# gstoica27/ReLUQP-py

Hardware: AMD Instinct MI355X
Metric: QP solves/sec (batch=4096 random dense QPs n=100 m=300) (higher is better)
Workload: dtype f32; 1 GPU; batch=4096/GPU random dense QPs n=100 m=300 (n_eq=25), feasible rand_qp seeds 0.., eps_abs=0.001, cold start, reference defaults; 4 distinct batches in rotation, every solve without dispatch history (= first solve of a fresh handle); global_batch=4096, parallelism=batch-split x1, no collectives, kernel=resident2, tile=same, low_memory=False, fresh_batches=4, dispatch_history=False, rho_window=5

## Files before the change

### reluqp-py_amd/csrc/rqp_resident2.hip

```cpp
#include <cstdio>
#include <cstdlib>
#include <type_traits>
#include <vector>

#include "rqp_common.h"

typedef float f2 __attribute__((ext_vector_type(2)));
typedef _Float16 h2 __attribute__((ext_vector_type(2)));

__device__ __forceinline__ float fma_mix_lo(h2 k, float v, float acc) {
    asm("v_fma_mix_f32 %0, %1, %2, %0 op_sel_hi:[1,0,0]" : "+v"(acc) : "v"(k), "v"(v));
    return acc;
}
__device__ __forceinline__ float fma_mix_hi(h2 k, float v, float acc) {
    asm("v_fma_mix_f32 %0, %1, %2, %0 op_sel:[1,0,0] op_sel_hi:[1,0,0]" : "+v"(acc) : "v"(k), "v"(v));
    return acc;
}
template <int CTRL>
__device__ __forceinline__ float dpp2(float v) {
    return __builtin_bit_cast(float, __builtin_amdgcn_update_dpp(0, __builtin_bit_cast(int, v), CTRL, 0xF, 0xF, true));
}
__device__ __forceinline__ float swsum32(float a, float b) {
    asm volatile("s_nop 1\n\tv_permlane32_swap_b32 %0, %1" : "+v"(a), "+v"(b));
    return a + b;
}
__device__ __forceinline__ float swsum16(float a, float b) {
    asm volatile("s_nop 1\n\tv_permlane16_swap_b32 %0, %1" : "+v"(a), "+v"(b));
    return a + b;
}
__device__ __forceinline__ float swmax32(float a, float b) {
    asm volatile("s_nop 1\n\tv_permlane32_swap_b32 %0, %1" : "+v"(a), "+v"(b));
    return fmaxf(a, b);
}
__device__ __forceinline__ float swmax16(float a, float b) {
    asm volatile("s_nop 1\n\tv_permlane16_swap_b32 %0, %1" : "+v"(a), "+v"(b));
    return fmaxf(a, b);
}
__device__ __forceinline__ float wave_max(float v) {
    v = fmaxf(v, dpp2<0xB1>(v));
    v = fmaxf(v, dpp2<0x4E>(v));
    v = fmaxf(v, dpp2<0x141>(v));
    v = fmaxf(v, dpp2<0x128>(v));
    float a = v, b = v;
    asm volatile("s_nop 1\n\tv_permlane16_swap_b32 %0, %1" : "+v"(a), "+v"(b));
    v = fmaxf(a, b);
    a = v; b = v;
    asm volatile("s_nop 1\n\tv_permlane32_swap_b32 %0, %1" : "+v"(a), "+v"(b));
    return fmaxf(a, b);
}
__device__ __forceinline__ unsigned wave_or(unsigned v) {
    v |= (unsigned)__builtin_amdgcn_update_dpp(0, (int)v, 0xB1, 0xF, 0xF, true);
    v |= (unsigned)__builtin_amdgcn_update_dpp(0, (int)v, 0x4E, 0xF, 0xF, true);
    v |= (unsigned)__builtin_amdgcn_update_dpp(0, (int)v, 0x141, 0xF, 0xF, true);
    v |= (unsigned)__builtin_amdgcn_update_dpp(0, (int)v, 0x128, 0xF, 0xF, true);
    unsigned a = v, b = v;
    asm volatile("s_nop 1\n\tv_permlane16_swap_b32 %0, %1" : "+v"(a), "+v"(b));
    v = a | b;
    a = v; b = v;
    asm volatile("s_nop 1\n\tv_permlane32_swap_b32 %0, %1" : "+v"(a), "+v"(b));
    return a | b;
}
template <typename T>
__device__ __forceinline__ T tmax2(T a, T b) {
    return (a != a) ? a : ((b != b) ? b : (a > b ? a : b));
}

template <int RB_, int CQ_, int KR_, int KC_>
struct Res2Cfg {
    static constexpr int RB = RB_, CQ = CQ_, KR = KR_, KC = KC_;
    static constexpr int NT = 256, NW = 4, NQ = 2, PL = 32;
    static constexpr int RP = RB / 2, KP = KR / 2;
    static constexpr int CW = NQ * CQ;
    static constexpr int N = NW * CW;
    static constexpr int M = PL * RB;
    static constexpr int SW = 8 * KR + 4;
    static constexpr int ND = NW * SW;
    static constexpr int AE2 = RP * CQ;
    static constexpr int KE2 = KP * KC;
    static constexpr int HR = 4, HP = HR / 2;
    static constexpr int HE2 = HP * CQ;
    static constexpr int HU = HE2 / 2;
    static constexpr int H1 = (CQ + 1) / 2, H2 = (H1 + 1) / 2;
    static constexpr int MATREGS = 2 * (RP * CQ + KP * KC);
    static constexpr int WAVES_PER_SIMD = (MATREGS > 100) ? 2 : ((MATREGS > 30) ? 3 : 4);
    static_assert(RB % 2 == 0 && KR % 2 == 0 && HP == 2 && HU == CQ && PL * HR >= N, "row pairs");
    static_assert(8 * KR >= CW && 8 * KC >= N && M <= 2 * NT && KC == CQ && NQ == 2, "tile shape");
    static constexpr size_t lds_bytes() {
        return (size_t)M * 8 * 4 + ND * 8 + 16 * 8
               + (size_t)M * 4 * 5
               + (size_t)ND * 4 * 6
               + (size_t)NW * M * 4 + 96 * 4
               + (size_t)HU * NT * 16;
    }
};

constexpr int NSEG = 25;
template <class C, bool DIAG, bool KH, bool KD = false>
__global__ void __launch_bounds__(256, C::WAVES_PER_SIMD) k_admm_res2(SolveArgs a, const float* __restrict__ Apack,
                                                      const float* __restrict__ Kpack,
                                                      const float* __restrict__ Hpack, unsigned long long* dbg,
                                                      const float* __restrict__ Kscale) {
    constexpr int RB = C::RB, CQ = C::CQ, KR = C::KR, KC = C::KC, NT = C::NT, NW = C::NW, RP = C::RP, KP = C::KP;
    constexpr int CW = C::CW, M = C::M, ND = C::ND, SW = C::SW, AE2 = C::AE2, KE2 = C::KE2, HU = C::HU, HP = C::HP, HR = C::HR, H1 = C::H1, H2 = C::H2;
    extern __shared__ __attribute__((aligned(16))) unsigned char smem_raw[];
    double* zt64 = (double*)smem_raw;
    double* lam64 = zt64 + M;
    double* z64 = lam64 + M;
    double* inv64 = z64 + M;
    double* x64 = inv64 + M;
    double* redd = x64 + ND;
    float* lT = (float*)(redd + 16);
    float* uT = lT + M;
    float* rv32 = uT + M;
    float* nu = rv32 + M;
    float* cT = nu + M;
    float* xin = cT + M;
    float* xnat = xin + ND;
    float* dxv = xnat + ND;
    float* hx = dxv + ND;
    float* gT = hx + ND;
    float* dvec = gT + ND;
    float* part = dvec + ND;
    float* red = part + NW * M;
    float* Hs = red + 96;
    static_assert(((size_t)M * 8 * 4 + ND * 8 + 16 * 8 + (size_t)M * 4 * 5 + ND * 4 * 6 + NW * M * 4 + 96 * 4) % 16 == 0,
                  "H image must start 16-byte aligned");

    const int n = a.n, m = a.m;
    const int b = a.order ? a.order[blockIdx.x] : (int)blockIdx.x, tid = threadIdx.x;
    const int wave = tid >> 6, lane = tid & 63;
    const int q = lane & 1, pl = lane >> 1, rr = lane >> 3, cc = lane & 7;
    const size_t mat = (a.sA == 0) ? 0 : (size_t)b;
    const float* cg = (const float*)a.c + (size_t)b * m;
    int k0 = 0;
    bool exact = false;
    if (a.cont == 1) {
        if (a.info.status[b] != RQP_STATUS_CONTINUE) {
            if (!(a.warm_starting || a.keep_state)) {
                for (int i = tid; i < n; i += NT) a.x[(size_t)b * n + i] = 0.0;
                for (int i = tid; i < m; i += NT) {
                    a.z[(size_t)b * m + i] = 0.0;
                    a.lam[(size_t)b * m + i] = 0.0;
                }
                if (tid == 0) a.rho_ind[b] = a.rho_ind0;
            }
            return;
        }
        k0 = a.cont_iter[b];
    } else if (a.cont == 2) {
        if (a.gate && *a.gate == 0) return;
        if (a.cstat[b] == 0) return;
        const int ci = a.cont_iter[b];
        if (ci >= 0) {
            k0 = ci;
            exact = true;
        }
    }
    const int wb = a.wbase ? a.wbase[mat] : 0;
    if (a.cstat && a.mode == 0) {
        const int sl = a.rho_ind[b] - wb;
        if (sl < 0 || sl >= a.kwin) {
            if (tid == 0) {
                a.cstat[b] = 1;
                if (!exact) a.cont_iter[b] = -1;
                atomicAdd(a.ncont, 1);
            }
            return;
        }
    }

    f2 ar[RP][CQ];
    {
        const f2* Ap = (const f2*)(Apack + mat * (size_t)AE2 * NT * 2) + tid;
#pragma unroll
        for (int rp = 0; rp < RP; ++rp)
#pragma unroll
            for (int c = 0; c < CQ; ++c) ar[rp][c] = Ap[(size_t)(rp * CQ + c) * NT];
        const float4* Hp = (const float4*)(Hpack + mat * (size_t)HU * NT * 4);
#pragma unroll
        for (int u = 0; u < HU; ++u) ((float4*)Hs)[u * NT + tid] = Hp[u * NT + tid];
    }
    int ri = a.rho_ind[b];
    float* rhoL = red + 64;
    if (tid < 32) rhoL[tid] = (tid < a.nrho) ? (float)a.rhos[tid] : 0.f;
    typedef typename std::conditional<KH, h2, f2>::type kpair_t;
    kpair_t kr[KP][KC];
    float kscale = 1.f;
    auto load_K = [&](int jl) {
        int j = jl - wb;
        j = j < 0 ? 0 : (j >= a.kwin ? a.kwin - 1 : j);
        if constexpr (!KD) {
            int tid_k = tid;
            asm volatile("" : "+v"(tid_k));
            const kpair_t* Kp = (const kpair_t*)Kpack + (mat * a.kwin + j) * (size_t)KE2 * NT + tid_k;
#pragma unroll
            for (int kp = 0; kp < KP; ++kp)
#pragma unroll
                for (int c = 0; c < KC; ++c) kr[kp][c] = Kp[(size_t)(kp * KC + c) * NT];
            if constexpr (KH) kscale = Kscale[mat * a.kwin + j];
        } else {
            int lane_o = lane, wave_o = wave;
            asm volatile("" : "+v"(lane_o), "+v"(wave_o));
            const int rr = lane_o >> 3, cc = lane_o & 7, wave = wave_o;
            const float* Kj = (const float*)a.K + ((a.sK == 0) ? (size_t)0 : (size_t)b * a.sK) + (size_t)j * n * a.ldn;
            typedef float f4u __attribute__((ext_vector_type(4), aligned(4)));
#pragma unroll
            for (int kp = 0; kp < KP; ++kp) {
                const int lr = KR * rr + 2 * kp, r = CW * wave + lr;
                const bool ok0 = lr < CW && r < n, ok1 = lr + 1 < CW && r + 1 < n;
                const float* row0 = Kj + (size_t)(r < n ? r : n - 1) * a.ldn + KC * cc;
                const float* row1 = Kj + (size_t)(r + 1 < n ? r + 1 : n - 1) * a.ldn + KC * cc;
                float t0[KC], t1[KC];
#pragma unroll
                for (int c = 0; c + 4 <= KC; c += 4) {
                    const f4u u0 = *(const f4u*)(row0 + c), u1 = *(const f4u*)(row1 + c);
#pragma unroll
                    for (int e = 0; e < 4; ++e) { t0[c + e] = u0[e]; t1[c + e] = u1[e]; }
                }
#pragma unroll
                for (int c = KC - KC % 4; c < KC; ++c) { t0[c] = row0[c]; t1[c] = row1[c]; }
                const f2 msk = {ok0 ? 1.f : 0.f, ok1 ? 1.f : 0.f};
#pragma unroll
                for (int c = 0; c < KC; ++c) kr[kp][c] = (f2){t0[c], t1[c]} * msk;
            }
        }
    };
    load_K(ri);

    auto set_rho_rows = [&](int j) {
        const float rho = (float)a.rhos[j];
        for (int i = tid; i < M; i += NT) {
            const float rv = rho * ((i < m) ? cg[i] : 1.f);
            rv32[i] = rv;
            inv64[i] = 1.0 / (double)rv;
        }
    };
    for (int i = tid; i < M; i += NT) {
        const bool in = i < m;
        zt64[i] = (exact && in) ? a.ax[(size_t)b * m + i] : 0.0;
        z64[i] = in ? a.z[(size_t)b * m + i] : 0.0;
        lam64[i] = in ? a.lam[(size_t)b * m + i] : 0.0;
        lT[i] = in ? ((const float*)a.l)[(size_t)b * m + i] : 0.f;
        uT[i] = in ? ((const float*)a.u)[(size_t)b * m + i] : 0.f;
        nu[i] = 0.f;
        cT[i] = in ? cg[i] : 1.f;
    }
    set_rho_rows(ri);
    for (int i = tid; i < ND; i += NT) {
        const int col = CW * (i / SW) + (i % SW);
        const bool in = (i % SW) < CW && col < n;
        const double xv = in ? a.x[(size_t)b * n + col] : 0.0;
        x64[i] = xv;
        xin[i] = (float)xv;
        xnat[i] = (i < n) ? (float)a.x[(size_t)b * n + i] : 0.f;
        gT[i] = in ? ((const float*)a.g)[(size_t)b * n + col] : 0.f;
        hx[i] = 0.f;
        dxv[i] = 0.f;
        dvec[i] = 0.f;
    }

    int colw, ncolw;
    {
        const int b5 = (lane >> 5) & 1, b4 = (lane >> 4) & 1;
        const int cbase = H2 * b4 + H1 * b5;
        int nval = b4 ? (H1 - H2) : H2;
        if (b5 && cbase + nval > CQ) nval = CQ - cbase;
        ncolw = ((lane & 0xE) == 0) ? nval : 0;
        colw = SW * wave + CQ * q + cbase;
    }
    __syncthreads();

    auto load_vc = [&](const float* v, float (&vc)[CQ]) __attribute__((always_inline)) {
#pragma unroll
        for (int c = 0; c < CQ; ++c) vc[c] = v[SW * wave + CQ * q + c];
    };
    auto prod_A = [&](const float (&vc)[CQ]) __attribute__((always_inline)) {
        f2 acc[RP];
#pragma unroll
        for (int rp = 0; rp < RP; ++rp) {
            f2 s = {0.f, 0.f};
#pragma unroll
            for (int c = 0; c < CQ; ++c) s = __builtin_elementwise_fma(ar[rp][c], (f2){vc[c], vc[c]}, s);
            s.x += dpp2<0xB1>(s.x);
            s.y += dpp2<0xB1>(s.y);
            acc[rp] = s;
        }
        if (q == 0) {
            f2* dst = (f2*)(part + wave * M + RB * pl);
#pragma unroll
            for (int rp = 0; rp < RP; ++rp) dst[rp] = acc[rp];
        }
    };
    auto prod_At = [&](auto use_a, auto use_h, const float* w, float* out, bool addg) {
        constexpr bool USE_A = decltype(use_a)::value, USE_H = decltype(use_h)::value;
        f2 wr[RP];
        f2 wx[HP];
        if constexpr (USE_A) {
#pragma unroll
            for (int rp = 0; rp < RP; ++rp) wr[rp] = ((const f2*)(w + RB * pl))[rp];
        }
        if constexpr (USE_H) {
            const float4 xv = *(const float4*)(xnat + HR * pl);
            wx[0] = (f2){xv.x, xv.y};
            wx[1] = (f2){xv.z, xv.w};
        }
        auto hload = [&](int c) -> float4 { return ((const float4*)Hs)[c * NT + tid]; };
        auto colsum = [&](int c, const float4& hv) -> float {
            f2 t2 = {0.f, 0.f};
            if constexpr (USE_A) {
#pragma unroll
                for (int rp = 0; rp < RP; ++rp) t2 = __builtin_elementwise_fma(ar[rp][c], wr[rp], t2);
            }
            if constexpr (USE_H) {
                t2 = __builtin_elementwise_fma((f2){hv.x, hv.y}, wx[0], t2);
                t2 = __builtin_elementwise_fma((f2){hv.z, hv.w}, wx[1], t2);
            }
            return t2.x + t2.y;
        };
        float s1[H1];
        auto colsum2 = [&](int c0, int c1, const float4& h0, const float4& h1, float& a0, float& a1) __attribute__((always_inline)) {
            f2 t0 = {0.f, 0.f}, t1 = {0.f, 0.f};
            if constexpr (USE_A) {
#pragma unroll
                for (int rp = 0; rp < RP; ++rp) {
                    t0 = __builtin_elementwise_fma(ar[rp][c0], wr[rp], t0);
                    t1 = __builtin_elementwise_fma(ar[rp][c1], wr[rp], t1);
                }
            }
            if constexpr (USE_H) {
                t0 = __builtin_elementwise_fma((f2){h0.x, h0.y}, wx[0], t0);
                t1 = __builtin_elementwise_fma((f2){h1.x, h1.y}, wx[0], t1);
                t0 = __builtin_elementwise_fma((f2){h0.z, h0.w}, wx[1], t0);
                t1 = __builtin_elementwise_fma((f2){h1.z, h1.w}, wx[1], t1);
            }
            a0 = t0.x + t0.y;
            a1 = t1.x + t1.y;
        };
        float4 hcur = {0.f, 0.f, 0.f, 0.f}, hnext = {0.f, 0.f, 0.f, 0.f};
        if constexpr (USE_H) {
            hcur = hload(0);
            if (H1 < CQ) hnext = hload(H1);
        }
#pragma unroll
        for (int i = 0; i < H1; ++i) {
            const bool pair = (i + H1 < CQ);
            if (pair) {
                float4 hc2 = hcur, hn2 = hnext;
                if constexpr (USE_H) {
                    if (i + 1 < H1) hc2 = hload(i + 1);
                    if (i + 1 + H1 < CQ) hn2 = hload(i + 1 + H1);
                }
                float a0, a1;
                colsum2(i, i + H1, hcur, hnext, a0, a1);
                s1[i] = swsum32(a0, a1);
                hcur = hc2;
                hnext = hn2;
            } else {
                const float a0 = colsum(i, hcur);
                s1[i] = swsum32(a0, a0);
            }
        }
        float gpre[H2];
#pragma unroll
        for (int i = 0; i < H2; ++i) gpre[i] = addg ? gT[colw + i] : 0.f;
        float s2[H2];
#pragma unroll
        for (int i = 0; i < H2; ++i) s2[i] = (i + H2 < H1) ? swsum16(s1[i], s1[i + H2]) : swsum16(s1[i], s1[i]);
#pragma unroll
        for (int i = 0; i < H2; ++i) {
            float v = s2[i];
            v += dpp2<0x4E>(v);
            v += dpp2<0x124>(v);
            v += dpp2<0x128>(v);
            s2[i] = v;
        }
        if (ncolw > 0) {
#pragma unroll
            for (int i = 0; i < H2; ++i)
                if (i < ncolw) out[colw + i] = s2[i] + gpre[i];
        }
    };
    constexpr std::true_type YES{};
    auto prod_At_chk = [&](const float* w, float* outA, float* outH) {
        f2 wr[RP];
        f2 wx[HP];
#pragma unroll
        for (int rp = 0; rp < RP; ++rp) wr[rp] = ((const f2*)(w + RB * pl))[rp];
        {
            const float4 xv = *(const float4*)(xnat + HR * pl);
            wx[0] = (f2){xv.x, xv.y};
            wx[1] = (f2){xv.z, xv.w};
        }
        auto hload = [&](int c) -> float4 { return ((const float4*)Hs)[c * NT + tid]; };
        float sA[H1], sH[H1];
        float4 hcur = hload(0), hnext = {0.f, 0.f, 0.f, 0.f};
        if (H1 < CQ) hnext = hload(H1);
#pragma unroll
        for (int i = 0; i < H1; ++i) {
            const bool pair = (i + H1 < CQ);
            float4 hc2 = hcur, hn2 = hnext;
            if (i + 1 < H1) hc2 = hload(i + 1);
            if (i + 1 + H1 < CQ) hn2 = hload(i + 1 + H1);
            f2 a0 = {0.f, 0.f}, a1 = {0.f, 0.f};
            f2 h0 = __builtin_elementwise_fma((f2){hcur.x, hcur.y}, wx[0], (f2){0.f, 0.f}), h1 = {0.f, 0.f};
            if (pair) h1 = __builtin_elementwise_fma((f2){hnext.x, hnext.y}, wx[0], h1);
#pragma unroll
            for (int rp = 0; rp < RP; ++rp) {
                a0 = __builtin_elementwise_fma(ar[rp][i], wr[rp], a0);
                if (pair) a1 = __builtin_elementwise_fma(ar[rp][i + H1], wr[rp], a1);
            }
            h0 = __builtin_elementwise_fma((f2){hcur.z, hcur.w}, wx[1], h0);
            if (pair) h1 = __builtin_elementwise_fma((f2){hnext.z, hnext.w}, wx[1], h1);
            const float ca0 = a0.x + a0.y, ch0 = h0.x + h0.y;
            sA[i] = pair ? swsum32(ca0, a1.x + a1.y) : swsum32(ca0, ca0);
            sH[i] = pair ? swsum32(ch0, h1.x + h1.y) : swsum32(ch0, ch0);
            hcur = hc2;
            hnext = hn2;
        }
        float tA[H2], tH[H2];
#pragma unroll
        for (int i = 0; i < H2; ++i) {
            tA[i] = (i + H2 < H1) ? swsum16(sA[i], sA[i + H2]) : swsum16(sA[i], sA[i]);
            tH[i] = (i + H2 < H1) ? swsum16(sH[i], sH[i + H2]) : swsum16(sH[i], sH[i]);
        }
#pragma unroll
        for (int i = 0; i < H2; ++i) {
            float va = tA[i], vh = tH[i];
            va += dpp2<0x4E>(va);
            vh += dpp2<0x4E>(vh);
            va += dpp2<0x124>(va);
            vh += dpp2<0x124>(vh);
            va += dpp2<0x128>(va);
            vh += dpp2<0x128>(vh);
            tA[i] = va;
            tH[i] = vh;
        }
        if (ncolw > 0) {
#pragma unroll
            for (int i = 0; i < H2; ++i)
                if (i < ncolw) {
                    outA[colw + i] = tA[i] + 0.f;
                    outH[colw + i] = tH[i] + 0.f;
                }
        }
    };
    auto prod_K = [&](const float* v, float (&s)[KR]) {
        float vc[KC];
#pragma unroll
        for (int c = 0; c < KC; ++c) vc[c] = v[SW * (cc >> 1) + CQ * (cc & 1) + c];
#pragma unroll
        for (int kp = 0; kp < KP; ++kp) {
            f2 t = {0.f, 0.f};
            if constexpr (KH) {
#pragma unroll
                for (int c = 0; c < KC; ++c) {
                    t.x = fma_mix_lo(kr[kp][c], vc[c], t.x);
                    t.y = fma_mix_hi(kr[kp][c], vc[c], t.y);
                }
                t.x *= kscale;
                t.y *= kscale;
            } else {
#pragma unroll
                for (int c = 0; c < KC; ++c) t = __builtin_elementwise_fma(kr[kp][c], (f2){vc[c], vc[c]}, t);
            }
            s[2 * kp] = t.x;
            s[2 * kp + 1] = t.y;
        }
#pragma unroll
        for (int r = 0; r < KR; ++r) s[r] += dpp2<0xB1>(s[r]);
#pragma unroll
        for (int r = 0; r < KR; ++r) s[r] += dpp2<0x4E>(s[r]);
#pragma unroll
        for (int r = 0; r < KR; ++r) s[r] += dpp2<0x141>(s[r]);
    };
    float cv[3] = {0.f, 0.f, 0.f};
    auto row_body = [&](auto nr, bool init, bool do_a, bool do_b, bool chk) __attribute__((always_inline)) {
        constexpr int R = decltype(nr)::value;
        double zt[R], z[R], lmv[R], iv[R];
        float adx[R][NW], lo[R], hi[R], rvf[R];
#pragma unroll
        for (int q = 0; q < R; ++q) {
            const int i = tid + q * NT;
            zt[q] = zt64[i];
            lmv[q] = lam64[i];
            if (do_a) {
                iv[q] = inv64[i];
                lo[q] = lT[i];
                hi[q] = uT[i];
            } else {
                z[q] = z64[i];
            }
            rvf[q] = rv32[i];
            if (init || do_a) {
#pragma unroll
                for (int w = 0; w < NW; ++w) adx[q][w] = part[w * M + i];
            }
        }
        asm volatile("s_waitcnt lgkmcnt(0)" ::: "memory");
#pragma unroll
        for (int q = 0; q < R; ++q) {
            asm volatile("" : "+v"(zt[q]), "+v"(lmv[q]), "+v"(rvf[q]));
            if (do_a) asm volatile("" : "+v"(iv[q]), "+v"(lo[q]), "+v"(hi[q]));
            else asm volatile("" : "+v"(z[q]));
            if (init || do_a) asm volatile("" : "+v"(adx[q][0]), "+v"(adx[q][1]), "+v"(adx[q][2]), "+v"(adx[q][3]));
        }
#pragma unroll
        for (int q = 0; q < R; ++q) {
            const int i = tid + q * NT;
            if (init || do_a) {
                const float ad = ((adx[q][0] + adx[q][1]) + adx[q][2]) + adx[q][3];
                zt[q] = (init ? 0.0 : zt[q]) + (double)ad;
                zt64[i] = zt[q];
            }
            if (do_a) {
                const double v = zt[q] + lmv[q] * iv[q];
                z[q] = v;
                if (v < (double)lo[q]) z[q] = (double)lo[q];
                if (v > (double)hi[q]) z[q] = (double)hi[q];
                z64[i] = z[q];
            }
            if (do_b) {
                const double rv = (double)rvf[q];
                const double pr = zt[q] - z[q];
                const double lh = lmv[q] + rv * pr;
                lam64[i] = lh;
                nu[i] = (float)(lh + rv * pr);
            }
        }
        if (chk) {
            int tid_w = tid;
            asm volatile("" : "+v"(tid_w));
#pragma unroll
            for (int q = 0; q < R; ++q) {
                const int i = tid_w + q * NT;
                const float we = (a.scE && i < m) ? (float)(1.0 / a.scE[mat * m + i]) : 1.f;
                nu[i] = (float)lmv[q];
                cv[0] = tmax2(cv[0], fabsf((float)(zt[q] - z[q])) * we);
                cv[1] = tmax2(cv[1], fabsf((float)zt[q]) * we);
                cv[2] = tmax2(cv[2], fabsf((float)z[q]) * we);
            }
        }
    };
    auto row_pass = [&](bool init, bool do_a, bool do_b, bool chk = false) __attribute__((always_inline)) {
        if constexpr (M > NT) {
            static_assert(M <= 2 * NT, "at most two rows per lane");
            if (tid + NT < M) {
                row_body(std::integral_constant<int, 2>{}, init, do_a, do_b, chk);
                return;
            }
        }
        if (tid < M) row_body(std::integral_constant<int, 1>{}, init, do_a, do_b, chk);
    };

    __builtin_amdgcn_s_waitcnt(0x0F70);
    unsigned long long t_last = 0, t_acc[NSEG] = {};
    bool k_pend = false;
    bool diag_on = true;
    auto stamp = [&](int seg) {
        if constexpr (DIAG) {
            __builtin_amdgcn_sched_barrier(0);
            unsigned long long t;
            asm volatile("s_memtime %0\n\ts_waitcnt lgkmcnt(0)" : "=s"(t)::"memory");
            __builtin_amdgcn_sched_barrier(0);
            if (seg >= 0 && diag_on) t_acc[seg] += t - t_last;
            t_last = t;
        }
    };

    float rho_est = (a.mode == 2) ? (float)a.rho_in : ((a.cont == 1 || exact) ? (float)a.cont_rho[b] : (float)a.rhos[ri]);
    float pri = 0.f, dua = 0.f;
    bool converged = false;
    int iters = k0;
    const float tolT = (float)a.tol;
    const int kmax = (a.mode == 2) ? 0 : a.max_iter;

    if (!exact) {
        float vc0[CQ];
        load_vc(xin, vc0);
        prod_A(vc0);
        __syncthreads();
        row_pass(true, false, kmax > k0);
    } else {
        row_pass(false, false, kmax > k0);
    }

    float scl_p = 0.f, scl_d = 0.f;
    auto res_rows = [&]() {
        cv[0] = cv[1] = cv[2] = 0.f;
        int tid_w = tid;
        asm volatile("" : "+v"(tid_w));
        for (int i = tid_w; i < M; i += NT) {
            const float we = (a.scE && i < m) ? (float)(1.0 / a.scE[mat * m + i]) : 1.f;
            nu[i] = (float)lam64[i];
            cv[0] = tmax2(cv[0], fabsf((float)(zt64[i] - z64[i])) * we);
            cv[1] = tmax2(cv[1], fabsf((float)zt64[i]) * we);
            cv[2] = tmax2(cv[2], fabsf((float)z64[i]) * we);
        }
    };
    int rpar = 0;
    auto residuals = [&](float rho_carry, float& o_pri, float& o_dua) -> float {
        float v[7];
#pragma unroll
        for (int e = 0; e < 3; ++e) v[e] = cv[e];
#pragma unroll
        for (int e = 3; e < 7; ++e) v[e] = 0.f;
        int tid_w = tid;
        asm volatile("" : "+v"(tid_w));
        __syncthreads();
        stamp(10);
        if (tid < ND && (tid % SW) >= CW) {
            dxv[tid] = 0.f;
            hx[tid] = 0.f;
        }
        prod_At_chk(nu, dxv, hx);
        stamp(11);
        __syncthreads();
        stamp(13);
        if (tid < ND) {
            float wd = 1.f;
            if (a.scD) {
                const int col = CW * (tid_w / SW) + (tid_w % SW);
                if ((tid_w % SW) < CW && col < n) wd = (float)(1.0 / (a.scC[mat] * a.scD[mat * n + col]));
            }
            const float t3 = dxv[tid];
            v[3] = fabsf(hx[tid] + t3 + gT[tid]) * wd;
            v[4] = fabsf(hx[tid]) * wd;
            v[5] = fabsf(t3) * wd;
            v[6] = fabsf(gT[tid]) * wd;
        }
        unsigned nanm = 0;
#pragma unroll
        for (int e = 0; e < 7; ++e) nanm |= (__builtin_amdgcn_ballot_w64(v[e] != v[e]) != 0ull) ? (1u << e) : 0u;
        float u0, u1;
        {
            const float r0 = swmax32(v[0], v[4]), r1 = swmax32(v[1], v[5]), r2 = swmax32(v[2], v[6]), r3 = swmax32(v[3], v[3]);
            u0 = swmax16(r0, r2);
            u1 = swmax16(r1, r3);
        }
        u0 = fmaxf(u0, dpp2<0xB1>(u0));
        u1 = fmaxf(u1, dpp2<0xB1>(u1));
        u0 = fmaxf(u0, dpp2<0x4E>(u0));
        u1 = fmaxf(u1, dpp2<0x4E>(u1));
        u0 = fmaxf(u0, dpp2<0x141>(u0));
        u1 = fmaxf(u1, dpp2<0x141>(u1));
        u0 = fmaxf(u0, dpp2<0x128>(u0));
        u1 = fmaxf(u1, dpp2<0x128>(u1));
        float* redp = red + 32 * rpar;
        rpar ^= 1;
        if ((lane & 15) == 0) {
            const int row = lane >> 4;
            *(f2*)(redp + wave * 8 + 2 * row) = (f2){u0, row == 3 ? __builtin_bit_cast(float, nanm) : u1};
        }
        stamp(14);
        __syncthreads();
        stamp(15);
        nanm = 0;
#pragma unroll
        for (int w = 0; w < NW; ++w) nanm |= __builtin_bit_cast(unsigned, redp[w * 8 + 7]);
#pragma unroll
        for (int e = 0; e < 7; ++e) {
            float r = redp[e];
#pragma unroll
            for (int w = 1; w < NW; ++w) r = fmaxf(r, redp[w * 8 + e]);
            v[e] = ((nanm >> e) & 1u) ? __builtin_nanf("") : r;
        }
        stamp(16);
        o_pri = v[0];
        o_dua = v[3];
        scl_p = tmax2(v[1], v[2]);
        scl_d = tmax2(tmax2(v[4], v[5]), v[6]);
        const float num = v[0] / scl_p;
        const float den = v[3] / scl_d;
        float est = rho_carry * sqrtf(num / den);
        if (est < (float)a.rho_min) est = (float)a.rho_min;
        if (est > (float)a.rho_max) est = (float)a.rho_max;
        return est;
    };

    stamp(-1);
    int to_chk = a.check_interval - (k0 % a.check_interval);
    for (int k = k0 + 1; k <= kmax; ++k) {
        __syncthreads();
        stamp(0);
        prod_At(YES, YES, nu, dvec, true);
        stamp(1);
        __syncthreads();
        stamp(2);
        __builtin_amdgcn_s_waitcnt(0x0F70);
        if constexpr (DIAG) {
            if (k_pend) { stamp(20); k_pend = false; }
        }
        {
            float s[KR];
            static_assert(KR == 4 || KR == 2, "vectorised x update");
            const int j = SW * wave + KR * rr;
            double2* xp = (double2*)(x64 + j);
            double2 xold[KR / 2];
#pragma unroll
            for (int hlf = 0; hlf < KR / 2; ++hlf) xold[hlf] = xp[hlf];
            prod_K(dvec, s);
            if (cc == 0) {
#pragma unroll
                for (int hlf = 0; hlf < KR / 2; ++hlf) ((f2*)(dxv + j))[hlf] = (f2){-s[2 * hlf], -s[2 * hlf + 1]};
            }
            __builtin_amdgcn_fence(__ATOMIC_RELEASE, "wavefront");
            __builtin_amdgcn_wave_barrier();
            float vc[CQ];
            load_vc(dxv, vc);
            if (cc == 0) {
                f2* xn2 = (f2*)(xnat + CW * wave + KR * rr);
#pragma unroll
                for (int hlf = 0; hlf < KR / 2; ++hlf) {
                    double2 xa = xold[hlf];
                    const f2 dx = {-s[2 * hlf], -s[2 * hlf + 1]};
                    xa.x += (double)dx.x;
                    xa.y += (double)dx.y;
                    xp[hlf] = xa;
                    const f2 xf = {(float)xa.x, (float)xa.y};
                    ((f2*)(xin + j))[hlf] = xf;
                    if (KR * rr + 2 * hlf + 1 < CW) xn2[hlf] = xf;
                }
            }
            stamp(3);
            prod_A(vc);
        }
        stamp(4);
        __syncthreads();
        stamp(5);
        stamp(6);
        iters = k;
        const bool on_grid = (--to_chk == 0);
        if (on_grid) to_chk = a.check_interval;
        const bool check = (a.mode == 0) && on_grid;
        if (!check) {
            row_pass(false, true, k < kmax);
            stamp(7);
        } else {
            cv[0] = cv[1] = cv[2] = 0.f;
            row_pass(false, true, false, true);
            stamp(8);
            if constexpr (DIAG) t_acc[22] += 1;
            const int ri_before = ri;
            rho_est = residuals(rho_est, pri, dua);
            rho_est = __builtin_bit_cast(float, __builtin_amdgcn_readfirstlane(__builtin_bit_cast(int, rho_est)));
            pri = __builtin_bit_cast(float, __builtin_amdgcn_readfirstlane(__builtin_bit_cast(int, pri)));
            dua = __builtin_bit_cast(float, __builtin_amdgcn_readfirstlane(__builtin_bit_cast(int, dua)));
            if (rho_est > rhoL[ri] * tolT && ri < a.nrho - 1)
                ri += 1;
            else if (rho_est < rhoL[ri] / tolT && ri > 0)
                ri -= 1;
            if (a.info.trace && (k / a.check_interval) <= a.info.trace_cap && tid == 0) {
                double* tr = a.info.trace + ((size_t)b * a.info.trace_cap + (k / a.check_interval - 1)) * 4;
                tr[0] = (double)pri; tr[1] = (double)dua; tr[2] = (double)rho_est; tr[3] = (double)ri_before;
            }
            float tp = (float)a.thr_p, td = (float)a.thr_d;
            if (a.eps_rel > 0) {
                tp += (float)a.eps_rel * __builtin_bit_cast(float, __builtin_amdgcn_readfirstlane(__builtin_bit_cast(int, scl_p)));
                td += (float)a.eps_rel * __builtin_bit_cast(float, __builtin_amdgcn_readfirstlane(__builtin_bit_cast(int, scl_d)));
            }
            stamp(18);
            if (pri < tp && dua < td) {
                converged = true;
                break;
            }
            if (ri != ri_before) {
                if (a.cstat && k < kmax && (ri < wb || ri >= wb + a.kwin)) {
                    int tid_o = tid;
                    asm volatile("" : "+v"(tid_o));
                    for (int i = tid_o; i < n; i += NT) a.x[(size_t)b * n + i] = x64[SW * (i / CW) + i % CW];
                    for (int i = tid_o; i < m; i += NT) {
                        a.z[(size_t)b * m + i] = z64[i];
                        a.lam[(size_t)b * m + i] = lam64[i];
                        a.ax[(size_t)b * m + i] = zt64[i];
                    }
                    if (tid_o == 0) {
                        a.rho_ind[b] = ri;
                        a.cont_iter[b] = k;
                        a.cont_rho[b] = (double)rho_est;
                        a.cstat[b] = 1;
                        atomicAdd(a.ncont, 1);
                    }
                    return;
                }
                if constexpr (DIAG) { t_acc[23] += 1; k_pend = true; }
                if constexpr (!KD) load_K(ri);
                {
                    int tid_o = tid;
                    asm volatile("" : "+v"(tid_o));
                    const float rho = rhoL[ri];
                    for (int i = tid_o; i < M; i += NT) {
                        const float rv = rho * cT[i];
                        rv32[i] = rv;
                        inv64[i] = 1.0 / (double)rv;
                    }
                }
                if constexpr (KD) load_K(ri);
                stamp(19);
            }
            if (k < kmax) row_pass(false, false, true);
            stamp(21);
        }
    }
    if constexpr (DIAG) {
        diag_on = false;
        if (lane == 0)
            for (int e = 0; e < NSEG; ++e) dbg[((size_t)b * 4 + wave) * NSEG + e] = (e == NSEG - 1) ? (unsigned long long)iters : t_acc[e];
    }

    __syncthreads();
    if (a.mode == 1) {
        for (int i = tid; i < n; i += NT) a.x[(size_t)b * n + i] = x64[SW * (i / CW) + i % CW];
        for (int i = tid; i < m; i += NT) {
            a.z[(size_t)b * m + i] = z64[i];
            a.lam[(size_t)b * m + i] = lam64[i];
        }
        return;
    }
    if (!converged) {
        res_rows();
        rho_est = residuals(rho_est, pri, dua);
    }

    double jp = 0.0;
    if (tid < ND) jp = (double)(xin[tid] * (0.5f * hx[tid] + gT[tid]));
    for (int off = 32; off >= 1; off >>= 1) jp += __shfl_xor(jp, off, 64);
    if (lane == 0) redd[wave] = jp;
    __syncthreads();
    const double obj = redd[0] + redd[1] + redd[2] + redd[3];

    if (a.mode == 2) {
        if (tid == 0) {
            if (a.r_pri) a.r_pri[b] = (double)pri;
            if (a.r_dua) a.r_dua[b] = (double)dua;
            if (a.r_rho) a.r_rho[b] = (double)rho_est;
            if (a.r_obj) a.r_obj[b] = obj;
        }
        return;
    }

    if (a.out_x) for (int i = tid; i < n; i += NT) ((float*)a.out_x)[(size_t)b * n + i] = (float)x64[SW * (i / CW) + i % CW];
    if (a.out_z) for (int i = tid; i < m; i += NT) ((float*)a.out_z)[(size_t)b * m + i] = (float)z64[i];
    if (a.out_lam) for (int i = tid; i < m; i += NT) ((float*)a.out_lam)[(size_t)b * m + i] = (float)lam64[i];
    if (tid == 0) {
        if (a.cstat) a.cstat[b] = 0;
        if (a.info.iter) a.info.iter[b] = converged ? iters : a.max_iter;
        if (a.last_iter) a.last_iter[b] = converged ? iters : a.max_iter;
        if (a.info.status) a.info.status[b] = converged ? RQP_STATUS_SOLVED : ((pri != pri || dua != dua) ? RQP_STATUS_NAN : RQP_STATUS_MAX_ITER);
        if (a.info.rho_ind) a.info.rho_ind[b] = ri;
        if (a.info.pri_res) a.info.pri_res[b] = (double)pri;
        if (a.info.dua_res) a.info.dua_res[b] = (double)dua;
        if (a.info.rho_estimate) a.info.rho_estimate[b] = (double)rho_est;
        if (a.info.obj_val) a.info.obj_val[b] = obj;
    }
    if ((a.warm_starting || a.keep_state)) {
        for (int i = tid; i < n; i += NT) a.x[(size_t)b * n + i] = x64[SW * (i / CW) + i % CW];
        for (int i = tid; i < m; i += NT) {
            a.z[(size_t)b * m + i] = z64[i];
            a.lam[(size_t)b * m + i] = lam64[i];
        }
        if (tid == 0) a.rho_ind[b] = ri;
    } else {
        for (int i = tid; i < n; i += NT) a.x[(size_t)b * n + i] = 0.0;
        for (int i = tid; i < m; i += NT) {
            a.z[(size_t)b * m + i] = 0.0;
            a.lam[(size_t)b * m + i] = 0.0;
        }
        if (tid == 0) a.rho_ind[b] = a.rho_ind0;
    }
}

template <class C, bool KH>
__global__ void k_pack_res2(int n, int ldn, int nrho, const float* __restrict__ K, float* __restrict__ Kpack, float* __restrict__ Kscale,
                            const int32_t* __restrict__ only, const int32_t* __restrict__ gate) {
    constexpr int KR = C::KR, KC = C::KC, NT = C::NT, CW = C::CW, KE2 = C::KE2;
    const int mat = blockIdx.y;
    if (gate && *gate == 0) return;
    if (only && !only[mat]) return;
    const int t = threadIdx.x, w = t >> 6, lane = t & 63;
    const int rr = lane >> 3, cc = lane & 7;
    extern __shared__ __attribute__((aligned(16))) float stage[];
    {
        const int j = blockIdx.x;
        const float* Kj = K + ((size_t)mat * nrho + j) * n * ldn;
        for (int i = t; i < n * ldn; i += NT) stage[i] = Kj[i];
        __syncthreads();
        float inv_scale = 1.f;
        if constexpr (KH) {
            __shared__ float smax[NT];
            float mx = 0.f;
            for (int i = t; i < n * ldn; i += NT) mx = fmaxf(mx, fabsf(stage[i]));
            smax[t] = mx;
            __syncthreads();
            for (int off = NT / 2; off >= 1; off >>= 1) {
                if (t < off) smax[t] = fmaxf(smax[t], smax[t + off]);
                __syncthreads();
            }
            int e2 = 0;
            (void)frexpf(fmaxf(smax[0], 1e-30f), &e2);
            const float sc = ldexpf(1.f, e2 - 14);
            inv_scale = ldexpf(1.f, 14 - e2);
            if (t == 0) Kscale[(size_t)mat * nrho + j] = sc;
        }
        float* Kp = Kpack + ((size_t)mat * nrho + j) * KE2 * NT * (KH ? 1 : 2);
        for (int pair = 0; pair < KE2; ++pair) {
            const int lr = KR * rr + 2 * (pair / KC);
            const int r = CW * w + lr, c = KC * cc + pair % KC;
            f2 v;
            v.x = (lr < CW && r < n && c < n) ? stage[r * ldn + c] : 0.f;
            v.y = (lr + 1 < CW && r + 1 < n && c < n) ? stage[(r + 1) * ldn + c] : 0.f;
            if constexpr (KH)
                ((h2*)Kp)[(size_t)pair * NT + t] = (h2){(_Float16)(v.x * inv_scale), (_Float16)(v.y * inv_scale)};
            else
                ((f2*)Kp)[(size_t)pair * NT + t] = v;
        }
    }
}


template <class C>
__global__ void k_pack_res2_ah(int n, int m, int ldn, const float* __restrict__ A, const float* __restrict__ Ht,
                               float* __restrict__ Apack, float* __restrict__ Hpack) {
    constexpr int RB = C::RB, CQ = C::CQ, NT = C::NT, CW = C::CW, AE2 = C::AE2, HU = C::HU, HR = C::HR, RCH = C::M / 4;
    const int mat = blockIdx.y, ch = blockIdx.x, t = threadIdx.x;
    extern __shared__ __attribute__((aligned(16))) float stage[];
    if (ch < 4) {
        if (!A) return;
        const int r0 = RCH * ch;
        const float* Am = A + (size_t)mat * m * ldn + (size_t)r0 * ldn;
        const int avail = (m - r0) * ldn;
        if ((((size_t)Am) & 15) == 0) {
            for (int i = 4 * t; i < RCH * ldn; i += 4 * NT)
                *(float4*)(stage + i) = (i < avail) ? *(const float4*)(Am + i) : (float4){0.f, 0.f, 0.f, 0.f};
        } else {
            for (int i = t; i < RCH * ldn; i += NT) stage[i] = (i < avail) ? Am[i] : 0.f;
        }
        __syncthreads();
        const int l16 = t & 15, w = (t >> 4) & 3, part = t >> 6;
        const int lane = 16 * ch + l16, q = lane & 1, pl = lane >> 1, tk = 64 * w + lane;
        f2* Ap = (f2*)(Apack + (size_t)mat * AE2 * NT * 2);
        for (int pair = part; pair < AE2; pair += 4) {
            const int lr = RB * pl + 2 * (pair / CQ) - r0, c = CW * w + CQ * q + pair % CQ;
            f2 v;
            v.x = (c < n) ? stage[lr * ldn + c] : 0.f;
            v.y = (c < n) ? stage[(lr + 1) * ldn + c] : 0.f;
            Ap[(size_t)pair * NT + tk] = v;
        }
    } else {
        const int w = t >> 6, lane = t & 63, q = lane & 1, pl = lane >> 1;
        const float* Hm = Ht + (size_t)mat * n * ldn;
        if ((((size_t)Hm) & 15) == 0) {
            for (int i = 4 * t; i < n * ldn; i += 4 * NT) *(float4*)(stage + i) = *(const float4*)(Hm + i);
        } else {
            for (int i = t; i < n * ldn; i += NT) stage[i] = Hm[i];
        }
        __syncthreads();
        float4* Hp = (float4*)(Hpack + (size_t)mat * HU * NT * 4);
        for (int c0 = 0; c0 < CQ; ++c0) {
            const int c = CW * w + CQ * q + c0;
            float hv[HR];
            for (int h = 0; h < HR; ++h) {
                const int r = HR * pl + h;
                hv[h] = (r < n && c < n) ? stage[c * ldn + r] : 0.f;
            }
            Hp[(size_t)c0 * NT + t] = (float4){hv[0], hv[1], hv[2], hv[3]};
        }
    }
}

typedef Res2Cfg<10, 13, 4, 13> Cfg2C2;
typedef Res2Cfg<2, 4, 2, 4> Cfg2C4;
typedef Res2Cfg<4, 7, 2, 7> Cfg2M;
typedef Res2Cfg<10, 10, 4, 10> Cfg2N;

static int res2_pick(const rqp_handle* h) {
    if (h->esz != 4 || h->nrho > 32) return -1;
    if (h->n <= Cfg2C4::N && h->m <= Cfg2C4::M) return 0;
    if (h->n <= Cfg2M::N && h->m <= Cfg2M::M) return 1;
    if (h->n <= Cfg2N::N && h->m <= Cfg2N::M) return 3;
    if (h->n <= Cfg2C2::N && h->m <= Cfg2C2::M) return 2;
    return -1;
}

bool rqp_res2_fits(const rqp_handle* h) { return res2_pick(h) >= 0; }

template <class C>
static void pack_elems_t(const rqp_handle* h, size_t* a_elems, size_t* k_elems, size_t* h_elems) {
    *a_elems = (size_t)h->nmat * C::AE2 * C::NT * 2;
    *k_elems = h->k_direct ? 0 : (size_t)h->nmat * h->kwin * C::KE2 * C::NT * (h->dims.tile_dtype == RQP_TILE_F16 ? 1 : 2);
    *h_elems = (size_t)h->nmat * C::HU * C::NT * 4;
}
void rqp_res2_pack_elems(const rqp_handle* h, size_t* a_elems, size_t* k_elems, size_t* h_elems) {
    switch (res2_pick(h)) {
        case 0: pack_elems_t<Cfg2C4>(h, a_elems, k_elems, h_elems); break;
        case 1: pack_elems_t<Cfg2M>(h, a_elems, k_elems, h_elems); break;
        case 3: pack_elems_t<Cfg2N>(h, a_elems, k_elems, h_elems); break;
        default: pack_elems_t<Cfg2C2>(h, a_elems, k_elems, h_elems); break;
    }
}

void rqp_res2_kp_layout(const rqp_handle* h, int* cw, int* kr, int* kc) {
    switch (res2_pick(h)) {
        case 0: *cw = Cfg2C4::CW; *kr = Cfg2C4::KR; *kc = Cfg2C4::KC; break;
        case 1: *cw = Cfg2M::CW; *kr = Cfg2M::KR; *kc = Cfg2M::KC; break;
        case 3: *cw = Cfg2N::CW; *kr = Cfg2N::KR; *kc = Cfg2N::KC; break;
        default: *cw = Cfg2C2::CW; *kr = Cfg2C2::KR; *kc = Cfg2C2::KC; break;
    }
}

template <class C>
static hipError_t pack_t(const rqp_handle* h, const void* A_src, const int32_t* only, const int32_t* gate, hipStream_t s) {
    const size_t stage_ah = (size_t)(C::M / 4 > h->n ? C::M / 4 : h->n) * h->ldn * sizeof(float);
    const size_t stage_k = (size_t)h->n * h->ldn * sizeof(float);
    if (!only)
        k_pack_res2_ah<C><<<dim3(5, h->nmat), C::NT, stage_ah, s>>>(h->n, h->m, h->ldn, (const float*)A_src, (const float*)h->Ht, h->Apack, h->Hpack);
    if (h->dims.tile_dtype == RQP_TILE_F16) {
        k_pack_res2<C, true><<<dim3(h->kwin, h->nmat), C::NT, stage_k, s>>>(h->n, h->ldn, h->kwin, (const float*)h->K, h->Kpack, h->Kscale, only, gate);
    } else {
        if (!h->k_direct && !h->kpack_direct)
            k_pack_res2<C, false><<<dim3(h->kwin, h->nmat), C::NT, stage_k, s>>>(h->n, h->ldn, h->kwin, (const float*)h->K, h->Kpack, nullptr, only, gate);
    }
    return hipGetLastError();
}
hipError_t rqp_launch_pack_res2(const rqp_handle* h, const void* A_src, const int32_t* only, const int32_t* gate, hipStream_t s) {
    switch (res2_pick(h)) {
        case 0: return pack_t<Cfg2C4>(h, A_src, only, gate, s);
        case 1: return pack_t<Cfg2M>(h, A_src, only, gate, s);
        case 3: return pack_t<Cfg2N>(h, A_src, only, gate, s);
        default: return pack_t<Cfg2C2>(h, A_src, only, gate, s);
    }
}

template <class C>
static hipError_t prepare_t(const rqp_handle* h) {
    const size_t lds = C::lds_bytes();
    {
        const size_t stage_ah = (size_t)(C::M / 4 > h->n ? C::M / 4 : h->n) * h->ldn * sizeof(float);
        hipError_t ae = rqp_raise_lds_limit((const void*)k_pack_res2_ah<C>, stage_ah);
        if (ae != hipSuccess) return ae;
    }
    {
        const size_t stage = (size_t)h->n * h->ldn * sizeof(float);
        hipError_t pe = (h->dims.tile_dtype == RQP_TILE_F16)
                            ? rqp_raise_lds_limit((const void*)k_pack_res2<C, true>, (size_t)stage)
                            : rqp_raise_lds_limit((const void*)k_pack_res2<C, false>, (size_t)stage);
        if (pe != hipSuccess) return pe;
    }
    if (h->dims.tile_dtype == RQP_TILE_F16)
        return rqp_raise_lds_limit((const void*)k_admm_res2<C, false, true>, (size_t)lds);
    hipError_t e = rqp_raise_lds_limit((const void*)k_admm_res2<C, false, false>, (size_t)lds);
    if (e != hipSuccess) return e;
    if (h->k_direct) {
        e = rqp_raise_lds_limit((const void*)k_admm_res2<C, false, false, true>, (size_t)lds);
        if (e != hipSuccess) return e;
    }
    if (h->debug & 2) e = rqp_raise_lds_limit((const void*)k_admm_res2<C, true, false>, (size_t)lds);
    if (h->debug & 1) {
        int nb = -1;
        hipError_t oe = hipOccupancyMaxActiveBlocksPerMultiprocessor(&nb, k_admm_res2<C, false, false>, C::NT, lds);
        hipFuncAttributes fa;
        (void)hipFuncGetAttributes(&fa, (const void*)k_admm_res2<C, false, false>);
        fprintf(stderr, "[rqp] k_admm_res2<%d,%d,%d,%d>: blocks/CU=%d (err %d) lds=%zu B regs=%d scratch=%zu B\n", C::RB, C::CQ,
                C::KR, C::KC, nb, (int)oe, lds, fa.numRegs, (size_t)fa.localSizeBytes);
    }
    return e;
}
hipError_t rqp_prepare_res2(const rqp_handle* h) {
    switch (res2_pick(h)) {
        case 0: return prepare_t<Cfg2C4>(h);
        case 1: return prepare_t<Cfg2M>(h);
        case 3: return prepare_t<Cfg2N>(h);
        default: return prepare_t<Cfg2C2>(h);
    }
}

template <class C>
static hipError_t solve_t(const rqp_handle* h, const SolveArgs& a, hipStream_t s) {
    const size_t lds = C::lds_bytes();
    if (h->dims.tile_dtype == RQP_TILE_F16) {
        k_admm_res2<C, false, true><<<h->B, C::NT, lds, s>>>(a, h->Apack, h->Kpack, h->Hpack, nullptr, h->Kscale);
        return hipGetLastError();
    }
    if ((h->debug & 2) && !h->k_direct) {
        const std::vector<double> sums = rqp_diag_run(s, h->B, 4, NSEG, [&](unsigned long long* dbg) {
            k_admm_res2<C, true, false><<<h->B, C::NT, lds, s>>>(a, h->Apack, h->Kpack, h->Hpack, dbg, nullptr);
        });
        if (sums.empty()) return hipErrorOutOfMemory;
        static const char* names[22] = {"B3 wait", "A'nu+Hx", "B1 wait", "Kd+x", "A dx", "B2 wait", "-", "rows",
                                        "rows(a)", "res rows", "R1 wait", "A'lam", "Hx", "R2 wait", "norms+reduce", "R3 wait", "combine",
                                        "R4 wait", "decision", "K issue+rho rows", "K wait", "rows(b)"};
        for (int w = 0; w < 4; ++w) {
            const double* tot = &sums[(size_t)w * NSEG];
            const double its = tot[NSEG - 1], chk = tot[22] > 0 ? tot[22] : 1.0;
            fprintf(stderr, "[rqp diag] wave %d cycles/iteration:", w);
            double sum = 0, csum = 0;
            for (int e = 8; e < 22; ++e) csum += tot[e];
            for (int e = 0; e < 8; ++e) { fprintf(stderr, " %s=%.0f", names[e], tot[e] / its); sum += tot[e] / its; }
            fprintf(stderr, " check=%.0f | total=%.0f\n", csum / its, sum + csum / its);
            fprintf(stderr, "[rqp diag] wave %d cycles/check:", w);
            for (int e = 8; e < 22; ++e) fprintf(stderr, " %s=%.0f", names[e], tot[e] / chk);
            fprintf(stderr, " | total=%.0f ; checks/instance=%.2f moves/instance=%.2f moves/check=%.3f\n", csum / chk, tot[22] / h->B,
                    tot[23] / h->B, tot[23] / chk);
        }
        return hipGetLastError();
    }
    if (h->k_direct)
        k_admm_res2<C, false, false, true><<<h->B, C::NT, lds, s>>>(a, h->Apack, nullptr, h->Hpack, nullptr, nullptr);
    else
        k_admm_res2<C, false, false><<<h->B, C::NT, lds, s>>>(a, h->Apack, h->Kpack, h->Hpack, nullptr, nullptr);
    return hipGetLastError();
}
hipError_t rqp_launch_solve_res2(const rqp_handle* h, const SolveArgs& a, hipStream_t s) {
    switch (res2_pick(h)) {
        case 0: return solve_t<Cfg2C4>(h, a, s);
        case 1: return solve_t<Cfg2M>(h, a, s);
        case 3: return solve_t<Cfg2N>(h, a, s);
        default: return solve_t<Cfg2C2>(h, a, s);
    }
}
```

Measured before the change: 1.412 million QP/s.

## Micro-optimize residual reduction, K reload addressing, and rho refresh in resident2

Several unrelated micro-optimizations land in the resident kernel. The K-register reload uses grouped byte offsets that fit immediate offset ranges. Equilibration weights are loaded before the row pass, and a cheaper NaN-propagating max is used. The cross-wave residual reduction is spread across lanes with DPP and readlane, and the rho up/down thresholds are precomputed in the same step. The rho refresh loop is also unrolled for two rows per lane. Each change targets instruction count or latency on the check and rho-change path, at the cost of more complex lane-specific code.

```diff
diff --git a/reluqp-py_amd/csrc/rqp_resident2.hip b/reluqp-py_amd/csrc/rqp_resident2.hip
--- a/reluqp-py_amd/csrc/rqp_resident2.hip
+++ b/reluqp-py_amd/csrc/rqp_resident2.hip
@@ -63,6 +63,15 @@
 template <typename T>
 __device__ __forceinline__ T tmax2(T a, T b) {
     return (a != a) ? a : ((b != b) ? b : (a > b ? a : b));
+}
+__device__ __forceinline__ float tmax2s(float a, float b) {
+    float r = (a > b) ? a : b;
+    r = (b != b) ? b : r;
+    r = (a != a) ? a : r;
+    return r;
+}
+__device__ __forceinline__ float lane_get(float v, int l) {
+    return __builtin_bit_cast(float, __builtin_amdgcn_readlane(__builtin_bit_cast(int, v), l));
 }
 
 template <int RB_, int CQ_, int KR_, int KC_>
@@ -192,11 +201,16 @@
         if constexpr (!KD) {
             int tid_k = tid;
             asm volatile("" : "+v"(tid_k));
-            const kpair_t* Kp = (const kpair_t*)Kpack + (mat * a.kwin + j) * (size_t)KE2 * NT + tid_k;
-#pragma unroll
-            for (int kp = 0; kp < KP; ++kp)
-#pragma unroll
-                for (int c = 0; c < KC; ++c) kr[kp][c] = Kp[(size_t)(kp * KC + c) * NT];
+            constexpr unsigned PB = (unsigned)sizeof(kpair_t) * NT, GP = 8192 / PB;
+            const char* Kb = (const char*)((const kpair_t*)Kpack + (mat * a.kwin + j) * (size_t)KE2 * NT);
+            const unsigned koff = (unsigned)tid_k * (unsigned)sizeof(kpair_t);
+#pragma unroll
+            for (unsigned g0 = 0; g0 < (unsigned)KE2; g0 += GP) {
+                const unsigned kg = koff + (g0 * PB + 4096u);
+#pragma unroll
+                for (unsigned p = g0; p < g0 + GP && p < (unsigned)KE2; ++p)
+                    kr[p / KC][p % KC] = *(const kpair_t*)(Kb + (size_t)kg + ((long)((p - g0) * PB) - 4096));
+            }
             if constexpr (KH) kscale = Kscale[mat * a.kwin + j];
         } else {
             int lane_o = lane, wave_o = wave;
@@ -478,6 +492,19 @@
         constexpr int R = decltype(nr)::value;
         double zt[R], z[R], lmv[R], iv[R];
         float adx[R][NW], lo[R], hi[R], rvf[R];
+        double sw[R];
+        bool wok[R];
+        const bool wts = chk && a.scE;
+        if (wts) {
+            int tid_w = tid;
+            asm volatile("" : "+v"(tid_w));
+#pragma unroll
+            for (int q = 0; q < R; ++q) {
+                const int i = tid_w + q * NT;
+                wok[q] = i < m;
+                sw[q] = wok[q] ? a.scE[mat * m + i] : 1.0;
+            }
+        }
 #pragma unroll
         for (int q = 0; q < R; ++q) {
             const int i = tid + q * NT;
@@ -530,14 +557,20 @@
         if (chk) {
             int tid_w = tid;
             asm volatile("" : "+v"(tid_w));
+            float we[R];
+#pragma unroll
+            for (int q = 0; q < R; ++q) we[q] = 1.f;
+            if (wts) {
+#pragma unroll
+                for (int q = 0; q < R; ++q) we[q] = wok[q] ? (float)(1.0 / sw[q]) : 1.f;
+            }
 #pragma unroll
             for (int q = 0; q < R; ++q) {
                 const int i = tid_w + q * NT;
-                const float we = (a.scE && i < m) ? (float)(1.0 / a.scE[mat * m + i]) : 1.f;
                 nu[i] = (float)lmv[q];
-                cv[0] = tmax2(cv[0], fabsf((float)(zt[q] - z[q])) * we);
-                cv[1] = tmax2(cv[1], fabsf((float)zt[q]) * we);
-                cv[2] = tmax2(cv[2], fabsf((float)z[q]) * we);
+                cv[0] = tmax2s(cv[0], fabsf((float)(zt[q] - z[q])) * we[q]);
+                cv[1] = tmax2s(cv[1], fabsf((float)zt[q]) * we[q]);
+                cv[2] = tmax2s(cv[2], fabsf((float)z[q]) * we[q]);
             }
         }
     };
@@ -585,6 +618,7 @@
     }
 
     float scl_p = 0.f, scl_d = 0.f;
+    float rho_up = 0.f, rho_dn = 0.f;
     auto res_rows = [&]() {
         cv[0] = cv[1] = cv[2] = 0.f;
         int tid_w = tid;
@@ -654,23 +688,45 @@
         stamp(14);
         __syncthreads();
         stamp(15);
-        nanm = 0;
-#pragma unroll
-        for (int w = 0; w < NW; ++w) nanm |= __builtin_bit_cast(unsigned, redp[w * 8 + 7]);
-#pragma unroll
-        for (int e = 0; e < 7; ++e) {
-            float r = redp[e];
-#pragma unroll
-            for (int w = 1; w < NW; ++w) r = fmaxf(r, redp[w * 8 + e]);
-            v[e] = ((nanm >> e) & 1u) ? __builtin_nanf("") : r;
-        }
+        const int lane_o = tid_w & 63, l8 = lane_o & 7, slot = l8 - (l8 >= 3 ? 1 : 0);
+        float rw[NW], mw[NW];
+#pragma unroll
+        for (int w = 0; w < NW; ++w) {
+            rw[w] = redp[w * 8 + slot];
+            mw[w] = redp[w * 8 + 7];
+        }
+        const float rl = rhoL[ri];
+        asm volatile("s_waitcnt lgkmcnt(0)" ::: "memory");
+#pragma unroll
+        for (int w = 0; w < NW; ++w) asm volatile("" : "+v"(rw[w]), "+v"(mw[w]));
+        float r = rw[0];
+        nanm = __builtin_bit_cast(unsigned, mw[0]);
+#pragma unroll
+        for (int w = 1; w < NW; ++w) {
+            r = fmaxf(r, rw[w]);
+            nanm |= __builtin_bit_cast(unsigned, mw[w]);
+        }
+        const float x = ((nanm >> slot) & 1u) ? __builtin_nanf("") : r;
         stamp(16);
-        o_pri = v[0];
-        o_dua = v[3];
-        scl_p = tmax2(v[1], v[2]);
-        scl_d = tmax2(tmax2(v[4], v[5]), v[6]);
-        const float num = v[0] / scl_p;
-        const float den = v[3] / scl_d;
+        float s = tmax2s(x, dpp2<0xE8>(x));
+        {
+            const float s3 = tmax2s(s, dpp2<0xEC>(x));
+            s = (lane_o & 4) ? s3 : s;
+        }
+        float qn = x, qd = dpp2<0xE5>(s);
+        if (lane_o == 8) {
+            qn = rl;
+            qd = tolT;
+        }
+        const float quo = qn / qd;
+        o_pri = lane_get(x, 0);
+        o_dua = lane_get(x, 4);
+        scl_p = lane_get(s, 1);
+        scl_d = lane_get(s, 5);
+        rho_dn = lane_get(quo, 8);
+        rho_up = rl * tolT;
+        const float num = lane_get(quo, 0);
+        const float den = lane_get(quo, 4);
         float est = rho_carry * sqrtf(num / den);
         if (est < (float)a.rho_min) est = (float)a.rho_min;
         if (est > (float)a.rho_max) est = (float)a.rho_max;
@@ -745,9 +801,9 @@
             rho_est = __builtin_bit_cast(float, __builtin_amdgcn_readfirstlane(__builtin_bit_cast(int, rho_est)));
             pri = __builtin_bit_cast(float, __builtin_amdgcn_readfirstlane(__builtin_bit_cast(int, pri)));
             dua = __builtin_bit_cast(float, __builtin_amdgcn_readfirstlane(__builtin_bit_cast(int, dua)));
-            if (rho_est > rhoL[ri] * tolT && ri < a.nrho - 1)
+            if (rho_est > rho_up && ri < a.nrho - 1)
                 ri += 1;
-            else if (rho_est < rhoL[ri] / tolT && ri > 0)
+            else if (rho_est < rho_dn && ri > 0)
                 ri -= 1;
             if (a.info.trace && (k / a.check_interval) <= a.info.trace_cap && tid == 0) {
                 double* tr = a.info.trace + ((size_t)b * a.info.trace_cap + (k / a.check_interval - 1)) * 4;
@@ -788,10 +844,25 @@
                     int tid_o = tid;
                     asm volatile("" : "+v"(tid_o));
                     const float rho = rhoL[ri];
-                    for (int i = tid_o; i < M; i += NT) {
-                        const float rv = rho * cT[i];
-                        rv32[i] = rv;
-                        inv64[i] = 1.0 / (double)rv;
+                    constexpr int RW = (M + NT - 1) / NT;
+                    if (RW == 2 && tid_o + NT < M) {
+                        float rv[2];
+                        double iv[2];
+#pragma unroll
+                        for (int q = 0; q < 2; ++q) rv[q] = rho * cT[tid_o + q * NT];
+#pragma unroll
+                        for (int q = 0; q < 2; ++q) iv[q] = 1.0 / (double)rv[q];
+#pragma unroll
+                        for (int q = 0; q < 2; ++q) {
+                            rv32[tid_o + q * NT] = rv[q];
+                            inv64[tid_o + q * NT] = iv[q];
+                        }
+                    } else {
+                        for (int i = tid_o; i < M; i += NT) {
+                            const float rv = rho * cT[i];
+                            rv32[i] = rv;
+                            inv64[i] = 1.0 / (double)rv;
+                        }
                     }
                 }
                 if constexpr (KD) load_K(ri);
```

Result: no change. 1.419 million QP/s (median of 6 runs) (+0.5%).
